# morrislab/rnascan

Measured on AMD Instinct MI355X. Metric: scored windows/sec (seq+struct, w=12), higher is better.
Workload: dtype f64

## Files before the change

### rnascan_amd/csrc/pfmscan_proflib.hip

```cpp
#include <float.h>
#include <math.h>

#include "pfmscan_internal.hpp"
#include "pfmscan_exact.hpp"
#include "pfmscan_hitqueue.hpp"

namespace pfmscan {

constexpr int PL_LANES = 256;
constexpr int PL_GROUPS = 4;
constexpr int PL_BLOCK = PL_LANES * PL_GROUPS;
#ifndef PL_V_OVERRIDE
#define PL_V_OVERRIDE 5
#endif
constexpr int PL_V = PL_V_OVERRIDE;
constexpr int PL_NS = PL_V + 1;
constexpr int PL_UNROLL = (PL_NS % 2) ? 2 * PL_NS : PL_NS;
constexpr int PL_TILE = PL_LANES * PL_V;
#ifndef PL_WAIT_FIRST
#define PL_WAIT_FIRST 1
#endif
#ifndef PL_STAGGER
#define PL_STAGGER 0
#endif
#ifndef PL_INTERLEAVE
#define PL_INTERLEAVE 0
#endif
constexpr int PL_QCAP = 128;

typedef uint32_t pl_u32x4 __attribute__((ext_vector_type(4)));
typedef double pl_f64x2 __attribute__((ext_vector_type(2)));

__device__ __forceinline__ double pl_nan_to_num(double d)
{
    double c = fmin(fmax(d, -DBL_MAX), DBL_MAX);
    return (d != d) ? 0.0 : c;
}

__host__ __device__ constexpr int pl_tile_vals(int m) { return ((PL_TILE + m) * 7 + 3) / 4 * 4; }
__host__ __device__ constexpr int pl_tile_bytes(int m) { return pl_tile_vals(m) * 8; }
__host__ __device__ constexpr int pl_queue_bytes() { return (PL_BLOCK / 64) * PL_QCAP * (8 + 4); }

__device__ __forceinline__ double pl_window_slow(const double *tile, int local, const double *__restrict__ pssm, int m)
{
    double score = 0.0;
#pragma unroll 1
    for (int j = 0; j < m; ++j) {
        const double *r = tile + (local + j) * 7;
        double d = r[0] * pssm[j * 7];
#pragma unroll 1
        for (int k = 1; k < 7; ++k) d = fma(r[k], pssm[j * 7 + k], d);
        score += pl_nan_to_num(d);
    }
    return score;
}

template <bool FINITE>
__device__ __forceinline__ void pl_score_motif(const double *tile, const double *__restrict__ pssm, const double *__restrict__ pssm_next,
                                               int m, int la, double (&acc)[PL_V], double (&P)[7])
{
    constexpr int V = PL_V, NS = PL_NS;
    const volatile __attribute__((address_space(3))) double *vt = (const volatile __attribute__((address_space(3))) double *)tile;
    double rows[NS][7];
#pragma unroll
    for (int s = 0; s < V; ++s) {
#pragma unroll
        for (int k = 0; k < 7; ++k) rows[s][k] = vt[(la + s) * 7 + k];
        acc[s] = 0.0;
    }
#if defined(PL_ABLATE) && (PL_ABLATE & 2)
#pragma unroll
    for (int k = 0; k < 7; ++k) rows[V][k] = rows[0][k];
#endif
    double Q[7];
    auto step = [&](const int uu, const int j) __attribute__((always_inline)) {
        const int u = uu % NS;
        double (&C)[7] = (uu & 1) ? Q : P;
        double (&N)[7] = (uu & 1) ? P : Q;
#if PL_WAIT_FIRST
        __builtin_amdgcn_s_waitcnt(0xC07F);
        __builtin_amdgcn_sched_barrier(0);
#endif
        const double *nrow = (j + 1 < m) ? pssm + (j + 1) * 7 : pssm_next;
        const __attribute__((address_space(4))) double *prow = (const __attribute__((address_space(4))) double *)nrow;
#if defined(PL_ABLATE) && (PL_ABLATE & 1)
        (void)prow;
#pragma unroll
        for (int k = 0; k < 7; ++k) N[k] = C[k];
#else
#pragma unroll
        for (int k = 0; k < 7; ++k) N[k] = prow[k];
#endif
#if defined(PL_ABLATE) && (PL_ABLATE & 2)
#else
#pragma unroll
        for (int k = 0; k < 7; ++k) rows[(u + V) % NS][k] = vt[(la + j + V) * 7 + k];
#endif
        if (FINITE) {
#pragma unroll
            for (int k = 0; k < 7; ++k) {
#pragma unroll
                for (int v = 0; v < V; ++v) acc[v] = fma(rows[(u + v) % NS][k], C[k], acc[v]);
            }
        } else {
#pragma unroll
            for (int v = 0; v < V; ++v) {
                const int slot = (u + v) % NS;
                double d = rows[slot][0] * C[0];
#pragma unroll
                for (int k = 1; k < 7; ++k) d = fma(rows[slot][k], C[k], d);
                acc[v] += pl_nan_to_num(d);
            }
        }
    };
    int j0 = 0;
#pragma unroll 1
    for (; j0 + PL_UNROLL <= m; j0 += PL_UNROLL) {
#pragma unroll
        for (int uu = 0; uu < PL_UNROLL; ++uu) step(uu, j0 + uu);
    }
#pragma unroll
    for (int uu = 0; uu < PL_UNROLL - 1; ++uu) {
        if (j0 + uu < m) step(uu, j0 + uu);
    }
    if (m & 1) {
#pragma unroll
        for (int k = 0; k < 7; ++k) P[k] = Q[k];
    }
    if (FINITE) {
#pragma unroll
        for (int v = 0; v < V; ++v)
            if (!(fabs(acc[v]) <= DBL_MAX)) acc[v] = pl_window_slow(tile, la + v, pssm, m);
    }
}

template <typename PROF_T>
__global__ __launch_bounds__(PL_BLOCK) void k_profile_lib(const ProfLibArgs a)
{
    constexpr int V = PL_V;
    constexpr int PER = 16 / (int)sizeof(PROF_T);
    typedef PROF_T vec_t __attribute__((ext_vector_type(PER)));
    extern __shared__ __align__(16) unsigned char smem[];
    const int m = a.m;
    double *tile = reinterpret_cast<double *>(smem);
    const int lane = threadIdx.x & 63;
    const int wave = __builtin_amdgcn_readfirstlane(threadIdx.x >> 6);
    const int group = wave / (PL_LANES / 64);
    double *q_sc = reinterpret_cast<double *>(smem + pl_tile_bytes(m)) + wave * PL_QCAP;
    uint32_t *q_wm = reinterpret_cast<uint32_t *>(smem + pl_tile_bytes(m) + (PL_BLOCK / 64) * PL_QCAP * 8) + wave * PL_QCAP;
    const int64_t n_pos = a.n_pos;
    const int64_t tile0 = (int64_t)blockIdx.x * PL_TILE;

    {
        const int nval = pl_tile_vals(m);
        const int64_t e0 = tile0 * 7, e_end = n_pos * 7;
        const PROF_T *__restrict__ src = reinterpret_cast<const PROF_T *>(a.profile) + e0;
        for (int i = threadIdx.x * PER; i < nval; i += PL_BLOCK * PER) {
            double d[PER];
            if (e0 + i + PER <= e_end) {
                const vec_t v = __builtin_nontemporal_load(reinterpret_cast<const vec_t *>(src + i));
#pragma unroll
                for (int e = 0; e < PER; ++e) d[e] = (double)v[e];
            } else {
#pragma unroll
                for (int e = 0; e < PER; ++e) d[e] = (e0 + i + e < e_end) ? (double)src[i + e] : 0.0;
            }
#pragma unroll
            for (int e = 0; e < PER; e += 2) *reinterpret_cast<pl_f64x2 *>(tile + i + e) = pl_f64x2{d[e], d[e + 1]};
        }
    }
    if (threadIdx.x < PL_LANES / 64)
        reinterpret_cast<uint32_t *>(smem + pl_tile_bytes(m) + pl_queue_bytes())[threadIdx.x] = PL_GROUPS;
    __syncthreads();
#if PL_STAGGER
    if (group == 1) __builtin_amdgcn_s_sleep(PL_STAGGER);
    if (group == 2) __builtin_amdgcn_s_sleep(2 * PL_STAGGER);
    if (group == 3) __builtin_amdgcn_s_sleep(3 * PL_STAGGER);
#endif

    const HitShard shard{a.hit_count, a.hit_shards, a.capacity};
    const unsigned long long shard_off = shard.off();
    int qn = 0;
    auto flush = [&]() {
        __builtin_amdgcn_fence(__ATOMIC_RELEASE, "wavefront");
        __builtin_amdgcn_wave_barrier();
        __builtin_amdgcn_fence(__ATOMIC_ACQUIRE, "wavefront");
        const unsigned long long base = shard.reserve_wave(qn);
        for (int i = lane; i < qn; i += 64) {
            const unsigned long long slot = base + (unsigned long long)i;
            if (shard.in_range(slot)) {
                const uint32_t wm = q_wm[i];
                a.hit_pos[shard_off + slot] = tile0 + (int64_t)(wm >> 16) + a.pos_offset;
                a.hit_motif[shard_off + slot] = a.motif_base + (int32_t)(wm & 0xFFFFu);
                a.hit_struct[shard_off + slot] = q_sc[i];
            }
        }
        __builtin_amdgcn_fence(__ATOMIC_RELEASE, "wavefront");
        __builtin_amdgcn_wave_barrier();
        qn = 0;
    };

    const int la = (threadIdx.x & (PL_LANES - 1)) * V;
    const int64_t live_all = n_pos - m + 1 - tile0;
    const int live_n = live_all < 0 ? 0 : (live_all > PL_TILE ? PL_TILE : (int)live_all);
    const __attribute__((address_space(4))) double *thr = (const __attribute__((address_space(4))) double *)a.thr;
    const __attribute__((address_space(4))) int32_t *finite = (const __attribute__((address_space(4))) int32_t *)a.finite;

    uint32_t *ticket = reinterpret_cast<uint32_t *>(smem + pl_tile_bytes(m) + pl_queue_bytes()) + (wave & (PL_LANES / 64 - 1));
    auto draw = [&]() -> uint32_t {
        uint32_t v = 0;
        if (lane == 0) v = atomicAdd(ticket, 1u);
        return v;
    };
    const int nm = a.n_motifs;
    int k = group;
    int kn = nm;
    double P[7];
    int fin = 0;
    if (k < nm) {
        const __attribute__((address_space(4))) double *p0 = (const __attribute__((address_space(4))) double *)(a.pssm + (size_t)k * m * 7);
#pragma unroll
        for (int c = 0; c < 7; ++c) P[c] = p0[c];
        fin = finite[k];
        kn = (int)__builtin_amdgcn_readfirstlane(draw());
    }
#pragma unroll 1
    while (k < nm) {
        const double *pssm = a.pssm + (size_t)k * m * 7;
        const int kc = kn < nm ? kn : k;
        const double *pssm_next = a.pssm + (size_t)kc * m * 7;
        const double t = thr[k];
        const int fin_next = finite[kc];
        double acc[V];
        if (fin)
            pl_score_motif<true>(tile, pssm, pssm_next, m, la, acc, P);
        else
            pl_score_motif<false>(tile, pssm, pssm_next, m, la, acc, P);
        fin = fin_next;
        const double t_lo = t - a.struct_band, t_hi = t + a.struct_band;
        bool maybe[V], any = false;
#pragma unroll
        for (int v = 0; v < V; ++v) {
            maybe[v] = (la + v < live_n) && (acc[v] > t_lo);
            any = any || maybe[v];
        }
        if (__builtin_expect(__builtin_amdgcn_ballot_w64(any) != 0, 0)) {
#pragma unroll
            for (int v = 0; v < V; ++v) {
                bool pass = maybe[v];
                if (__builtin_amdgcn_ballot_w64(pass) == 0) continue;
                if (pass && acc[v] <= t_hi) {
                    acc[v] = struct_window_rounded(tile + (la + v) * 7, m, [&](int j, int c) { return pssm[j * 7 + c]; });
                    pass = acc[v] > t;
                }
                const unsigned long long mk = __builtin_amdgcn_ballot_w64(pass);
                if (mk) {
                    if (qn + 64 > PL_QCAP) flush();
                    if (pass) {
                        const int slot = qn + (int)__builtin_amdgcn_mbcnt_hi((uint32_t)(mk >> 32), __builtin_amdgcn_mbcnt_lo((uint32_t)mk, 0u));
                        q_sc[slot] = acc[v];
                        q_wm[slot] = ((uint32_t)(la + v) << 16) | (uint32_t)k;
                    }
                    qn += __popcll(mk);
                }
            }
        }
        k = kn;
        if (kn < nm) kn = (int)__builtin_amdgcn_readfirstlane(draw());
    }
    if (qn > 0) flush();
}

int64_t profile_library_tile() { return PL_TILE; }

hipError_t launch_profile_library(const ProfLibArgs &a, hipStream_t stream)
{
    if (a.n_pos <= 0 || a.n_motifs <= 0) return hipSuccess;
    if (a.n_motifs > 65536 || a.m < 1 || a.m > PFMSCAN_MAX_M) return hipErrorInvalidValue;
    const unsigned grid = (unsigned)((a.n_pos + PL_TILE - 1) / PL_TILE);
    const size_t lds = (size_t)pl_tile_bytes(a.m) + pl_queue_bytes() + 16;
    static std::atomic<uint64_t> done_f{0}, done_d{0};
    if (a.profile_dtype == PFMSCAN_PROFILE_F64) {
        hipError_t e = allow_dynamic_lds(reinterpret_cast<const void *>(k_profile_lib<double>), done_d, 160 * 1024);
        if (e != hipSuccess) return e;
        hipLaunchKernelGGL(k_profile_lib<double>, dim3(grid), dim3(PL_BLOCK), lds, stream, a);
    } else {
        hipError_t e = allow_dynamic_lds(reinterpret_cast<const void *>(k_profile_lib<float>), done_f, 160 * 1024);
        if (e != hipSuccess) return e;
        hipLaunchKernelGGL(k_profile_lib<float>, dim3(grid), dim3(PL_BLOCK), lds, stream, a);
    }
    return hipGetLastError();
}

}
```

Measured before the change: 148.9 billion.

## Score motif pairs per tile pass with width-specialized kernels

Motifs are now processed in pairs, so each LDS profile row loaded into registers feeds two motifs' FMAs. This halves the LDS row traffic per motif when both are finite. The kernel is templated on motif width (1-15), which fully unrolls the column loop. The per-window non-finite check moves from the hot path into the emit path, guarded by a block-level flag set when the tile holds out-of-range values. The cost is more registers per thread, which could lower occupancy or cause spills, plus more kernel instantiations.

```diff
diff --git a/rnascan_amd/csrc/pfmscan_proflib.hip b/rnascan_amd/csrc/pfmscan_proflib.hip
--- a/rnascan_amd/csrc/pfmscan_proflib.hip
+++ b/rnascan_amd/csrc/pfmscan_proflib.hip
@@ -17,16 +17,20 @@
 constexpr int PL_NS = PL_V + 1;
 constexpr int PL_UNROLL = (PL_NS % 2) ? 2 * PL_NS : PL_NS;
 constexpr int PL_TILE = PL_LANES * PL_V;
-#ifndef PL_WAIT_FIRST
-#define PL_WAIT_FIRST 1
-#endif
-#ifndef PL_STAGGER
-#define PL_STAGGER 0
-#endif
-#ifndef PL_INTERLEAVE
-#define PL_INTERLEAVE 0
+#ifndef PL_PAIRS
+#define PL_PAIRS 1
+#endif
+#ifndef PL_FIXED_WIDTHS
+#define PL_FIXED_WIDTHS 1
+#endif
+#ifndef PL_FIXED_WIDTH_LIST
+#define PL_FIXED_WIDTH_LIST                                                                                               \
+    PL_WIDTH(1) PL_WIDTH(2) PL_WIDTH(3) PL_WIDTH(4) PL_WIDTH(5) PL_WIDTH(6) PL_WIDTH(7) PL_WIDTH(8) PL_WIDTH(9) PL_WIDTH(10) \
+    PL_WIDTH(11) PL_WIDTH(12) PL_WIDTH(13) PL_WIDTH(14) PL_WIDTH(15)
 #endif
 constexpr int PL_QCAP = 128;
+constexpr int PL_TICKET_BYTES = 16;
+constexpr int PL_FLAG_BYTES = (PL_BLOCK / 64) * 4;
 
 typedef uint32_t pl_u32x4 __attribute__((ext_vector_type(4)));
 typedef double pl_f64x2 __attribute__((ext_vector_type(2)));
@@ -55,102 +59,111 @@
     return score;
 }
 
-template <bool FINITE>
-__device__ __forceinline__ void pl_score_motif(const double *tile, const double *__restrict__ pssm, const double *__restrict__ pssm_next,
-                                               int m, int la, double (&acc)[PL_V], double (&P)[7])
-{
+template <bool FINITE, int NM, int M>
+__device__ __forceinline__ void pl_score(const double *tile, const double *__restrict__ pssm, const double *__restrict__ nextA,
+                                         const double *__restrict__ nextB, int m_rt, int la, double (&accA)[PL_V], double (&accB)[PL_V],
+                                         double (&PA)[7], double (&PB)[7])
+{
+    static_assert(NM == 1 || (NM == 2 && FINITE), "the pair form exists for all-finite motifs only");
     constexpr int V = PL_V, NS = PL_NS;
+    const int m = M ? M : m_rt;
     const volatile __attribute__((address_space(3))) double *vt = (const volatile __attribute__((address_space(3))) double *)tile;
     double rows[NS][7];
+    const volatile __attribute__((address_space(3))) double *vl = vt + la * 7;
 #pragma unroll
     for (int s = 0; s < V; ++s) {
 #pragma unroll
-        for (int k = 0; k < 7; ++k) rows[s][k] = vt[(la + s) * 7 + k];
-        acc[s] = 0.0;
-    }
-#if defined(PL_ABLATE) && (PL_ABLATE & 2)
-#pragma unroll
-    for (int k = 0; k < 7; ++k) rows[V][k] = rows[0][k];
-#endif
-    double Q[7];
-    auto step = [&](const int uu, const int j) __attribute__((always_inline)) {
+        for (int k = 0; k < 7; ++k) rows[s][k] = vl[s * 7 + k];
+        accA[s] = 0.0;
+        if (NM == 2) accB[s] = 0.0;
+    }
+    double QA[7], QB[7];
+    auto step = [&](const int uu, const int j, const volatile __attribute__((address_space(3))) double *g) __attribute__((always_inline)) {
         const int u = uu % NS;
-        double (&C)[7] = (uu & 1) ? Q : P;
-        double (&N)[7] = (uu & 1) ? P : Q;
-#if PL_WAIT_FIRST
+        double (&CA)[7] = (uu & 1) ? QA : PA;
+        double (&NA)[7] = (uu & 1) ? PA : QA;
+        double (&CB)[7] = (uu & 1) ? QB : PB;
+        double (&NB)[7] = (uu & 1) ? PB : QB;
         __builtin_amdgcn_s_waitcnt(0xC07F);
         __builtin_amdgcn_sched_barrier(0);
-#endif
-        const double *nrow = (j + 1 < m) ? pssm + (j + 1) * 7 : pssm_next;
+        const double *nrow = (j + 1 < m) ? pssm + (j + 1) * 7 : nextA;
         const __attribute__((address_space(4))) double *prow = (const __attribute__((address_space(4))) double *)nrow;
-#if defined(PL_ABLATE) && (PL_ABLATE & 1)
-        (void)prow;
-#pragma unroll
-        for (int k = 0; k < 7; ++k) N[k] = C[k];
-#else
-#pragma unroll
-        for (int k = 0; k < 7; ++k) N[k] = prow[k];
-#endif
-#if defined(PL_ABLATE) && (PL_ABLATE & 2)
-#else
-#pragma unroll
-        for (int k = 0; k < 7; ++k) rows[(u + V) % NS][k] = vt[(la + j + V) * 7 + k];
-#endif
+#pragma unroll
+        for (int k = 0; k < 7; ++k) NA[k] = prow[k];
+        if (NM == 2) {
+            const double *nrow_b = (j + 1 < m) ? pssm + (m + j + 1) * 7 : nextB;
+            const __attribute__((address_space(4))) double *prow_b = (const __attribute__((address_space(4))) double *)nrow_b;
+#pragma unroll
+            for (int k = 0; k < 7; ++k) NB[k] = prow_b[k];
+        }
+#pragma unroll
+        for (int k = 0; k < 7; ++k) rows[(u + V) % NS][k] = g[(uu + V) * 7 + k];
         if (FINITE) {
 #pragma unroll
             for (int k = 0; k < 7; ++k) {
 #pragma unroll
-                for (int v = 0; v < V; ++v) acc[v] = fma(rows[(u + v) % NS][k], C[k], acc[v]);
+                for (int v = 0; v < V; ++v) {
+                    accA[v] = fma(rows[(u + v) % NS][k], CA[k], accA[v]);
+                    if (NM == 2) accB[v] = fma(rows[(u + v) % NS][k], CB[k], accB[v]);
+                }
             }
         } else {
 #pragma unroll
             for (int v = 0; v < V; ++v) {
                 const int slot = (u + v) % NS;
-                double d = rows[slot][0] * C[0];
-#pragma unroll
-                for (int k = 1; k < 7; ++k) d = fma(rows[slot][k], C[k], d);
-                acc[v] += pl_nan_to_num(d);
-            }
-        }
-    };
-    int j0 = 0;
-#pragma unroll 1
-    for (; j0 + PL_UNROLL <= m; j0 += PL_UNROLL) {
-#pragma unroll
-        for (int uu = 0; uu < PL_UNROLL; ++uu) step(uu, j0 + uu);
-    }
-#pragma unroll
-    for (int uu = 0; uu < PL_UNROLL - 1; ++uu) {
-        if (j0 + uu < m) step(uu, j0 + uu);
+                double d = rows[slot][0] * CA[0];
+#pragma unroll
+                for (int k = 1; k < 7; ++k) d = fma(rows[slot][k], CA[k], d);
+                accA[v] += pl_nan_to_num(d);
+            }
+        }
+    };
+    if (M > 0) {
+#pragma unroll
+        for (int uu = 0; uu < (M > 0 ? M : 1); ++uu) step(uu, uu, vl);
+    } else {
+        int j0 = 0;
+#pragma unroll 1
+        for (; j0 + PL_UNROLL <= m; j0 += PL_UNROLL) {
+            const volatile __attribute__((address_space(3))) double *g = vl + j0 * 7;
+#pragma unroll
+            for (int uu = 0; uu < PL_UNROLL; ++uu) step(uu, j0 + uu, g);
+        }
+        const volatile __attribute__((address_space(3))) double *g = vl + j0 * 7;
+#pragma unroll
+        for (int uu = 0; uu < PL_UNROLL - 1; ++uu) {
+            if (j0 + uu < m) step(uu, j0 + uu, g);
+        }
     }
     if (m & 1) {
 #pragma unroll
-        for (int k = 0; k < 7; ++k) P[k] = Q[k];
-    }
-    if (FINITE) {
-#pragma unroll
-        for (int v = 0; v < V; ++v)
-            if (!(fabs(acc[v]) <= DBL_MAX)) acc[v] = pl_window_slow(tile, la + v, pssm, m);
-    }
-}
-
-template <typename PROF_T>
+        for (int k = 0; k < 7; ++k) {
+            PA[k] = QA[k];
+            if (NM == 2) PB[k] = QB[k];
+        }
+    }
+}
+
+template <typename PROF_T, int M>
 __global__ __launch_bounds__(PL_BLOCK) void k_profile_lib(const ProfLibArgs a)
 {
     constexpr int V = PL_V;
     constexpr int PER = 16 / (int)sizeof(PROF_T);
     typedef PROF_T vec_t __attribute__((ext_vector_type(PER)));
     extern __shared__ __align__(16) unsigned char smem[];
-    const int m = a.m;
+    const int m = M ? M : a.m;
     double *tile = reinterpret_cast<double *>(smem);
     const int lane = threadIdx.x & 63;
     const int wave = __builtin_amdgcn_readfirstlane(threadIdx.x >> 6);
     const int group = wave / (PL_LANES / 64);
     double *q_sc = reinterpret_cast<double *>(smem + pl_tile_bytes(m)) + wave * PL_QCAP;
     uint32_t *q_wm = reinterpret_cast<uint32_t *>(smem + pl_tile_bytes(m) + (PL_BLOCK / 64) * PL_QCAP * 8) + wave * PL_QCAP;
+    uint32_t *tickets = reinterpret_cast<uint32_t *>(smem + pl_tile_bytes(m) + pl_queue_bytes());
+    uint32_t *flags = reinterpret_cast<uint32_t *>(smem + pl_tile_bytes(m) + pl_queue_bytes() + PL_TICKET_BYTES);
     const int64_t n_pos = a.n_pos;
     const int64_t tile0 = (int64_t)blockIdx.x * PL_TILE;
 
+    bool odd_entry = false;
     {
         const int nval = pl_tile_vals(m);
         const int64_t e0 = tile0 * 7, e_end = n_pos * 7;
@@ -166,22 +179,32 @@
                 for (int e = 0; e < PER; ++e) d[e] = (e0 + i + e < e_end) ? (double)src[i + e] : 0.0;
             }
 #pragma unroll
+            for (int e = 0; e < PER; ++e) odd_entry = odd_entry || !(fabs(d[e]) <= STRUCT_ROW_MAX);
+#pragma unroll
             for (int e = 0; e < PER; e += 2) *reinterpret_cast<pl_f64x2 *>(tile + i + e) = pl_f64x2{d[e], d[e + 1]};
         }
     }
     if (threadIdx.x < PL_LANES / 64)
-        reinterpret_cast<uint32_t *>(smem + pl_tile_bytes(m) + pl_queue_bytes())[threadIdx.x] = PL_GROUPS;
+        tickets[threadIdx.x] = PL_GROUPS;
+    {
+        const bool odd_wave = __builtin_amdgcn_ballot_w64(odd_entry) != 0;
+        if (lane == 0) flags[wave] = odd_wave ? 1u : 0u;
+    }
     __syncthreads();
-#if PL_STAGGER
-    if (group == 1) __builtin_amdgcn_s_sleep(PL_STAGGER);
-    if (group == 2) __builtin_amdgcn_s_sleep(2 * PL_STAGGER);
-    if (group == 3) __builtin_amdgcn_s_sleep(3 * PL_STAGGER);
-#endif
-
-    const HitShard shard{a.hit_count, a.hit_shards, a.capacity};
-    const unsigned long long shard_off = shard.off();
+    const bool force = __builtin_amdgcn_ballot_w64(lane < PL_BLOCK / 64 && flags[lane & (PL_BLOCK / 64 - 1)] != 0) != 0 ||
+                       !(a.struct_band <= 0x1p900);
+
     int qn = 0;
     auto flush = [&]() {
+        const __attribute__((address_space(4))) ProfLibArgs *ap = (const __attribute__((address_space(4))) ProfLibArgs *)__builtin_amdgcn_kernarg_segment_ptr();
+        asm volatile("" : "+s"(ap));
+        const HitShard shard{ap->hit_count, ap->hit_shards, ap->capacity};
+        const unsigned long long shard_off = shard.off();
+        const int64_t pos0 = (int64_t)blockIdx.x * PL_TILE + ap->pos_offset;
+        const int32_t motif_base = ap->motif_base;
+        int64_t *const hit_pos = ap->hit_pos;
+        int32_t *const hit_motif = ap->hit_motif;
+        double *const hit_struct = ap->hit_struct;
         __builtin_amdgcn_fence(__ATOMIC_RELEASE, "wavefront");
         __builtin_amdgcn_wave_barrier();
         __builtin_amdgcn_fence(__ATOMIC_ACQUIRE, "wavefront");
@@ -190,9 +213,9 @@
             const unsigned long long slot = base + (unsigned long long)i;
             if (shard.in_range(slot)) {
                 const uint32_t wm = q_wm[i];
-                a.hit_pos[shard_off + slot] = tile0 + (int64_t)(wm >> 16) + a.pos_offset;
-                a.hit_motif[shard_off + slot] = a.motif_base + (int32_t)(wm & 0xFFFFu);
-                a.hit_struct[shard_off + slot] = q_sc[i];
+                hit_pos[shard_off + slot] = pos0 + (int64_t)(wm >> 16);
+                hit_motif[shard_off + slot] = motif_base + (int32_t)(wm & 0xFFFFu);
+                hit_struct[shard_off + slot] = q_sc[i];
             }
         }
         __builtin_amdgcn_fence(__ATOMIC_RELEASE, "wavefront");
@@ -200,96 +223,150 @@
         qn = 0;
     };
 
-    const int la = (threadIdx.x & (PL_LANES - 1)) * V;
+    const int la_hot = (threadIdx.x & (PL_LANES - 1)) * V;
     const int64_t live_all = n_pos - m + 1 - tile0;
     const int live_n = live_all < 0 ? 0 : (live_all > PL_TILE ? PL_TILE : (int)live_all);
     const __attribute__((address_space(4))) double *thr = (const __attribute__((address_space(4))) double *)a.thr;
     const __attribute__((address_space(4))) int32_t *finite = (const __attribute__((address_space(4))) int32_t *)a.finite;
 
-    uint32_t *ticket = reinterpret_cast<uint32_t *>(smem + pl_tile_bytes(m) + pl_queue_bytes()) + (wave & (PL_LANES / 64 - 1));
+    auto screen = [&](const double (&acc)[V], const double t, bool (&cand)[V]) __attribute__((always_inline)) -> unsigned long long {
+        const double t_lo = t - a.struct_band;
+        bool any = force;
+#pragma unroll
+        for (int v = 0; v < V; ++v) {
+            cand[v] = !(acc[v] <= t_lo);
+            any = any || cand[v];
+        }
+        return __builtin_amdgcn_ballot_w64(any);
+    };
+    auto emit = [&](const int k, double (&acc)[V], const bool (&cand)[V], const double t, const double *pssm, const bool fin) __attribute__((always_inline)) {
+        const double t_lo = t - a.struct_band, t_hi = t + a.struct_band;
+        int la = la_hot;
+        asm volatile("" : "+v"(la));
+#pragma unroll
+        for (int v = 0; v < V; ++v) {
+            bool pass = (force || cand[v]) && (la + v < live_n);
+            if (__builtin_amdgcn_ballot_w64(pass) == 0) continue;
+            if (fin && pass && !(fabs(acc[v]) <= DBL_MAX)) acc[v] = pl_window_slow(tile, la + v, pssm, m);
+            pass = pass && acc[v] > t_lo;
+            if (pass && acc[v] <= t_hi) {
+                acc[v] = struct_window_rounded(tile + (la + v) * 7, m, [&](int j, int c) { return pssm[j * 7 + c]; });
+                pass = acc[v] > t;
+            }
+            const unsigned long long mk = __builtin_amdgcn_ballot_w64(pass);
+            if (mk) {
+                if (qn + 64 > PL_QCAP) flush();
+                if (pass) {
+                    const int slot = qn + (int)__builtin_amdgcn_mbcnt_hi((uint32_t)(mk >> 32), __builtin_amdgcn_mbcnt_lo((uint32_t)mk, 0u));
+                    q_sc[slot] = acc[v];
+                    q_wm[slot] = ((uint32_t)(la + v) << 16) | (uint32_t)k;
+                }
+                qn += __popcll(mk);
+            }
+        }
+    };
+
+    uint32_t *ticket = tickets + (wave & (PL_LANES / 64 - 1));
     auto draw = [&]() -> uint32_t {
         uint32_t v = 0;
         if (lane == 0) v = atomicAdd(ticket, 1u);
         return v;
     };
     const int nm = a.n_motifs;
-    int k = group;
-    int kn = nm;
-    double P[7];
-    int fin = 0;
-    if (k < nm) {
-        const __attribute__((address_space(4))) double *p0 = (const __attribute__((address_space(4))) double *)(a.pssm + (size_t)k * m * 7);
-#pragma unroll
-        for (int c = 0; c < 7; ++c) P[c] = p0[c];
-        fin = finite[k];
-        kn = (int)__builtin_amdgcn_readfirstlane(draw());
-    }
-#pragma unroll 1
-    while (k < nm) {
-        const double *pssm = a.pssm + (size_t)k * m * 7;
-        const int kc = kn < nm ? kn : k;
-        const double *pssm_next = a.pssm + (size_t)kc * m * 7;
-        const double t = thr[k];
-        const int fin_next = finite[kc];
-        double acc[V];
-        if (fin)
-            pl_score_motif<true>(tile, pssm, pssm_next, m, la, acc, P);
-        else
-            pl_score_motif<false>(tile, pssm, pssm_next, m, la, acc, P);
-        fin = fin_next;
-        const double t_lo = t - a.struct_band, t_hi = t + a.struct_band;
-        bool maybe[V], any = false;
-#pragma unroll
-        for (int v = 0; v < V; ++v) {
-            maybe[v] = (la + v < live_n) && (acc[v] > t_lo);
-            any = any || maybe[v];
-        }
-        if (__builtin_expect(__builtin_amdgcn_ballot_w64(any) != 0, 0)) {
-#pragma unroll
-            for (int v = 0; v < V; ++v) {
-                bool pass = maybe[v];
-                if (__builtin_amdgcn_ballot_w64(pass) == 0) continue;
-                if (pass && acc[v] <= t_hi) {
-                    acc[v] = struct_window_rounded(tile + (la + v) * 7, m, [&](int j, int c) { return pssm[j * 7 + c]; });
-                    pass = acc[v] > t;
-                }
-                const unsigned long long mk = __builtin_amdgcn_ballot_w64(pass);
-                if (mk) {
-                    if (qn + 64 > PL_QCAP) flush();
-                    if (pass) {
-                        const int slot = qn + (int)__builtin_amdgcn_mbcnt_hi((uint32_t)(mk >> 32), __builtin_amdgcn_mbcnt_lo((uint32_t)mk, 0u));
-                        q_sc[slot] = acc[v];
-                        q_wm[slot] = ((uint32_t)(la + v) << 16) | (uint32_t)k;
-                    }
-                    qn += __popcll(mk);
-                }
-            }
-        }
-        k = kn;
-        if (kn < nm) kn = (int)__builtin_amdgcn_readfirstlane(draw());
+    const int units = (nm + 1) >> 1;
+    int u = group;
+    int un = units;
+    double PA[7], PB[7];
+    int fin_a = 0, fin_b = 0;
+    if (u < units) {
+        const int k0 = 2 * u, k1 = k0 + 1 < nm ? k0 + 1 : k0;
+        const __attribute__((address_space(4))) double *p0 = (const __attribute__((address_space(4))) double *)(a.pssm + (size_t)k0 * m * 7);
+        const __attribute__((address_space(4))) double *p1 = (const __attribute__((address_space(4))) double *)(a.pssm + (size_t)k1 * m * 7);
+#pragma unroll
+        for (int c = 0; c < 7; ++c) {
+            PA[c] = p0[c];
+            PB[c] = p1[c];
+        }
+        fin_a = finite[k0];
+        fin_b = finite[k1];
+        un = (int)__builtin_amdgcn_readfirstlane(draw());
+    }
+#pragma unroll 1
+    while (u < units) {
+        const int k0 = 2 * u;
+        const int here = k0 + 1 < nm ? 2 : 1;
+        const double *pssm = a.pssm + (size_t)k0 * m * 7;
+        const int uc = un < units ? un : u;
+        const int n0 = 2 * uc, n1 = n0 + 1 < nm ? n0 + 1 : n0;
+        const double *next_a = a.pssm + (size_t)n0 * m * 7, *next_b = a.pssm + (size_t)n1 * m * 7;
+        const double t_a = thr[k0], t_b = thr[k0 + here - 1];
+        const int fin_a_next = finite[n0], fin_b_next = finite[n1];
+        double acc_a[V], acc_b[V];
+        if (PL_PAIRS && M > 0 && here == 2 && fin_a && fin_b) {
+            pl_score<true, 2, M>(tile, pssm, next_a, next_b, m, la_hot, acc_a, acc_b, PA, PB);
+            bool cand_a[V], cand_b[V];
+            const unsigned long long any_a = screen(acc_a, t_a, cand_a), any_b = screen(acc_b, t_b, cand_b);
+            if (__builtin_expect(any_a != 0, 0)) emit(k0, acc_a, cand_a, t_a, pssm, true);
+            if (__builtin_expect(any_b != 0, 0)) emit(k0 + 1, acc_b, cand_b, t_b, pssm + m * 7, true);
+        } else {
+#pragma unroll 1
+            for (int s = 0; s < here; ++s) {
+                const double *ps = pssm + (size_t)s * m * 7;
+                const double *nx = s + 1 < here ? ps + m * 7 : next_a;
+                const int fin = s ? fin_b : fin_a;
+                if (fin)
+                    pl_score<true, 1, 0>(tile, ps, nx, nx, m, la_hot, acc_a, acc_b, PA, PB);
+                else
+                    pl_score<false, 1, 0>(tile, ps, nx, nx, m, la_hot, acc_a, acc_b, PA, PB);
+                const double t = s ? t_b : t_a;
+                bool cand[V];
+                if (__builtin_expect(screen(acc_a, t, cand) != 0, 0)) emit(k0 + s, acc_a, cand, t, ps, fin != 0);
+            }
+            const __attribute__((address_space(4))) double *p1 = (const __attribute__((address_space(4))) double *)next_b;
+#pragma unroll
+            for (int c = 0; c < 7; ++c) PB[c] = p1[c];
+        }
+        fin_a = fin_a_next;
+        fin_b = fin_b_next;
+        u = un;
+        if (un < units) un = (int)__builtin_amdgcn_readfirstlane(draw());
     }
     if (qn > 0) flush();
 }
 
 int64_t profile_library_tile() { return PL_TILE; }
+
+template <typename PROF_T, int M>
+static hipError_t launch_lib_width(const ProfLibArgs &a, hipStream_t stream)
+{
+    const unsigned grid = (unsigned)((a.n_pos + PL_TILE - 1) / PL_TILE);
+    const size_t lds = (size_t)pl_tile_bytes(a.m) + pl_queue_bytes() + PL_TICKET_BYTES + PL_FLAG_BYTES;
+    static std::atomic<uint64_t> done{0};
+    hipError_t e = allow_dynamic_lds(reinterpret_cast<const void *>(k_profile_lib<PROF_T, M>), done, 160 * 1024);
+    if (e != hipSuccess) return e;
+    hipLaunchKernelGGL((k_profile_lib<PROF_T, M>), dim3(grid), dim3(PL_BLOCK), lds, stream, a);
+    return hipGetLastError();
+}
+
+template <typename PROF_T>
+static hipError_t launch_lib(const ProfLibArgs &a, hipStream_t stream)
+{
+#if PL_FIXED_WIDTHS
+    switch (a.m) {
+#define PL_WIDTH(W) case W: return launch_lib_width<PROF_T, W>(a, stream);
+        PL_FIXED_WIDTH_LIST
+#undef PL_WIDTH
+    default: break;
+    }
+#endif
+    return launch_lib_width<PROF_T, 0>(a, stream);
+}
 
 hipError_t launch_profile_library(const ProfLibArgs &a, hipStream_t stream)
 {
     if (a.n_pos <= 0 || a.n_motifs <= 0) return hipSuccess;
     if (a.n_motifs > 65536 || a.m < 1 || a.m > PFMSCAN_MAX_M) return hipErrorInvalidValue;
-    const unsigned grid = (unsigned)((a.n_pos + PL_TILE - 1) / PL_TILE);
-    const size_t lds = (size_t)pl_tile_bytes(a.m) + pl_queue_bytes() + 16;
-    static std::atomic<uint64_t> done_f{0}, done_d{0};
-    if (a.profile_dtype == PFMSCAN_PROFILE_F64) {
-        hipError_t e = allow_dynamic_lds(reinterpret_cast<const void *>(k_profile_lib<double>), done_d, 160 * 1024);
-        if (e != hipSuccess) return e;
-        hipLaunchKernelGGL(k_profile_lib<double>, dim3(grid), dim3(PL_BLOCK), lds, stream, a);
-    } else {
-        hipError_t e = allow_dynamic_lds(reinterpret_cast<const void *>(k_profile_lib<float>), done_f, 160 * 1024);
-        if (e != hipSuccess) return e;
-        hipLaunchKernelGGL(k_profile_lib<float>, dim3(grid), dim3(PL_BLOCK), lds, stream, a);
-    }
-    return hipGetLastError();
-}
-
-}
+    return a.profile_dtype == PFMSCAN_PROFILE_F64 ? launch_lib<double>(a, stream) : launch_lib<float>(a, stream);
+}
+
+}
```

Result: no change. 148.4 billion (-0.4%).
